# Lightning-AI/lit-llama

Hardware: NVIDIA H100
Metric: LLaMA-7B gptq.int4 decode tokens/sec (higher is better)
Workload: dtype bf16

## Files before the change

### lit-llama_b200/csrc/attention.cu

```cuda
#include <cstdlib>

#include "b2l_common.cuh"

namespace b2l {

__global__ void ring_advance_kernel(const int64_t* __restrict__ input_pos, int T, int32_t* ring_start, int S) {
  if (threadIdx.x == 0 && blockIdx.x == 0) {
    if (input_pos[T - 1] >= (int64_t)S) *ring_start = (*ring_start + 1) % S;
  }
}

__global__ void rope_append_kernel(__nv_bfloat16* __restrict__ qkv, __nv_bfloat16* __restrict__ k_cache,
                                   __nv_bfloat16* __restrict__ v_cache, const float* __restrict__ rope,
                                   const int64_t* __restrict__ input_pos, const int32_t* __restrict__ ring_start,
                                   int T, int n_head, int hs, int S, int block_size, int rope_rows) {
  const int bt = blockIdx.x, h = blockIdx.y, b = bt / T, t = bt % T;
  const int C = n_head * hs;
  long long p = input_pos ? input_pos[t] : (long long)t;
  const long long prow = rope_rows ? (long long)t : (p < block_size ? p : (long long)block_size - 1);
  __nv_bfloat16* q = qkv + (size_t)bt * 3 * C + h * hs;
  __nv_bfloat16* k = q + C;
  const __nv_bfloat16* v = q + 2 * C;
  __nv_bfloat16 *kd = k, *vd = nullptr;
  if (k_cache != nullptr) {
// ... 77 lines not shown
    } else {
#pragma unroll
      for (int e = 0; e < ATT_MAX_EPL; ++e) {
        int d = lane + 32 * e;
        kx[e] = d < hs ? bf2f(kr[d]) : 0.f;
        vx[e] = d < hs ? bf2f(vr[d]) : 0.f;
      }
    }
    float sc = 0.f;
#pragma unroll
    for (int e = 0; e < (EPL > 0 ? EPL : ATT_MAX_EPL); ++e) sc = fmaf(qv[e], kx[e], sc);
    sc = warp_sum(sc);
    const float mn = fmaxf(m, sc);
    const float corr = __expf(m - mn), pj = __expf(sc - mn);
    l = l * corr + pj;
#pragma unroll
    for (int e = 0; e < (EPL > 0 ? EPL : ATT_MAX_EPL); ++e) acc[e] = fmaf(pj, vx[e], acc[e] * corr);
    m = mn;
  }
  __shared__ float sm_m[ATT_WARPS], sm_l[ATT_WARPS];
  __shared__ float sm_acc[ATT_WARPS][32 * ATT_MAX_EPL];
  if (lane == 0) { sm_m[warp] = m; sm_l[warp] = l; }
#pragma unroll
  for (int e = 0; e < (EPL > 0 ? EPL : ATT_MAX_EPL); ++e) {
    int d = (EPL > 0) ? lane * EPL + e : lane + 32 * e;
    sm_acc[warp][d] = acc[e];
  }
  __syncthreads();
  float M = -INFINITY;
#pragma unroll
  for (int w = 0; w < ATT_WARPS; ++w) M = fmaxf(M, sm_m[w]);
  float Ls = 0.f;
  float wgt[ATT_WARPS];
#pragma unroll
  for (int w = 0; w < ATT_WARPS; ++w) {
    wgt[w] = (sm_m[w] == -INFINITY) ? 0.f : __expf(sm_m[w] - M);
    Ls += sm_l[w] * wgt[w];
  }
  if (threadIdx.x == 0) { out[0] = M; out[1] = Ls; }
  for (int d = threadIdx.x; d < hs; d += blockDim.x) {
    float a = 0.f;
#pragma unroll
    for (int w = 0; w < ATT_WARPS; ++w) a += sm_acc[w][d] * wgt[w];
    out[2 + d] = a;
  }
}

__global__ void attn_combine_kernel(const float* __restrict__ work, __nv_bfloat16* __restrict__ y, int T,
                                    int n_head, int hs, int n_split) {
  pdl_launch_dependents();
  const int bh = blockIdx.x, b = bh / n_head, h = bh % n_head, t = blockIdx.y;
  const float* base = work + ((size_t)bh * T + t) * n_split * (hs + 2);
  float M = -INFINITY;
  for (int s = 0; s < n_split; ++s) M = fmaxf(M, base[(size_t)s * (hs + 2)]);
  float Ls = 0.f;
  for (int s = 0; s < n_split; ++s) {
    float ms = base[(size_t)s * (hs + 2)];
    if (ms != -INFINITY) Ls += base[(size_t)s * (hs + 2) + 1] * __expf(ms - M);
  }
  const float inv = 1.0f / Ls;
  __nv_bfloat16* yr = y + ((size_t)b * T + t) * (n_head * hs) + h * hs;
  for (int d = threadIdx.x; d < hs; d += blockDim.x) {
    float a = 0.f;
    for (int s = 0; s < n_split; ++s) {
      float ms = base[(size_t)s * (hs + 2)];
      if (ms != -INFINITY) a += base[(size_t)s * (hs + 2) + 2 + d] * __expf(ms - M);
    }
    yr[d] = f2bf(a * inv);
  }
}

__global__ void kv_unroll_kernel(const __nv_bfloat16* __restrict__ cache, const int32_t* __restrict__ ring_start,
                                 __nv_bfloat16* __restrict__ out, int S, int hs) {
  const int ring = *ring_start;
  const int phys = (blockIdx.y + ring) % S;
  const __nv_bfloat16* src = cache + ((size_t)blockIdx.x * S + phys) * hs;
  __nv_bfloat16* dst = out + ((size_t)blockIdx.x * S + blockIdx.y) * hs;
  for (int d = threadIdx.x; d < hs; d += blockDim.x) dst[d] = src[d];
}

constexpr int FD_CHUNK = 256;
constexpr int FD_SUB = 64;
constexpr int FD_WARPS = 8;
constexpr int FD_CTAS_PER_SM = 3;
constexpr int WS_CHUNK = FD_SUB;

__device__ __forceinline__ void bf16x8_to_f32(const uint4& u, float* f) {
  const uint32_t w[4] = {u.x, u.y, u.z, u.w};
#pragma unroll
  for (int i = 0; i < 4; ++i) {
    f[2 * i] = __uint_as_float(w[i] << 16);
    f[2 * i + 1] = __uint_as_float(w[i] & 0xffff0000u);
  }
}

__device__ __forceinline__ uint32_t fd_smem_u32(const void* p) { return (uint32_t)__cvta_generic_to_shared(p); }
__device__ __forceinline__ void fd_bulk(uint32_t dst, const void* src, uint32_t bytes, uint32_t bar) {
  asm volatile("cp.async.bulk.shared::cluster.global.mbarrier::complete_tx::bytes [%0], [%1], %2, [%3];" ::"r"(dst), "l"(src), "r"(bytes), "r"(bar) : "memory");
}

constexpr int FD_SUB_BYTES = FD_SUB * 128 * 2;
constexpr int FD_SMEM_BYTES = 4 * FD_SUB_BYTES + FD_WARPS * 128 * 4 + 2 * FD_WARPS * 4 + 16;

__global__ void __launch_bounds__(FD_WARPS * 32)
    attn_decode_fused_kernel(const __nv_bfloat16* qkv, __nv_bfloat16* __restrict__ k_cache,
                             __nv_bfloat16* __restrict__ v_cache, const float* __restrict__ rope,
                             const int64_t* __restrict__ input_pos, const int32_t* __restrict__ ring_start,
                             __nv_bfloat16* __restrict__ y, float* __restrict__ work, int* __restrict__ tickets,
                             int n_head, int S, int block_size, int n_split, unsigned long long* tl, int pre_tiles,
                             int smem_merge, int target_ctas) {
  constexpr int HS = 128;
  extern __shared__ __align__(128) uint8_t fsm[];
  float* sm_acc = reinterpret_cast<float*>(fsm + 4 * FD_SUB_BYTES);
  float* sm_m = sm_acc + FD_WARPS * HS;
  float* sm_l = sm_m + FD_WARPS;
  unsigned long long* bars = reinterpret_cast<unsigned long long*>(sm_l + FD_WARPS);
  __shared__ int sm_last;

  if (threadIdx.x == 0) tl_min(tl, 0);
  const int bh = blockIdx.x, b = bh / n_head, h = bh % n_head, sp = blockIdx.y;
  unsigned long long* tl0 = (tl != nullptr && blockIdx.x == 0 && blockIdx.y == 0 && threadIdx.x == 0) ? tl + 8 : nullptr;
  int tli = 0;
  auto stamp = [&]() { if (tl0 != nullptr && tli < 24) tl0[tli++] = globaltimer_ns(); };
  stamp();
  const int lane = threadIdx.x & 31, warp = threadIdx.x >> 5;
  const int C = n_head * HS;
  const size_t head_base = ((size_t)b * n_head + h) * S * HS;

  const long long p = input_pos[0];
  const int w_slot = (int)(p < S ? p : (long long)S - 1);
  const int L = w_slot + 1;
  const int want_splits = max(1, target_ctas / (int)gridDim.x);
  const int chunk = L <= FD_CHUNK ? FD_CHUNK
                                  : min(FD_CHUNK, max(FD_SUB, FD_SUB * ((L + FD_SUB * want_splits - 1) / (FD_SUB * want_splits))));
  const int n_active = (L + chunk - 1) / chunk;
  if (sp >= n_active) return;
  const int ring = *ring_start;
  const int j0 = sp * chunk, j1 = min(L, j0 + chunk);
  const int n_old = min(j1, L - 1) - j0;
  const int n_sub = (n_old + FD_SUB - 1) / FD_SUB;
  const bool has_new = (w_slot >= j0 && w_slot < j1);

  const uint32_t bar0 = fd_smem_u32(bars);
  auto request = [&](int i) {
    const int buf = i & 1;
    const int cnt = min(FD_SUB, n_old - i * FD_SUB);
    int phys0 = j0 + i * FD_SUB + ring; if (phys0 >= S) phys0 -= S;
    const int first = min(cnt, S - phys0);
    const uint32_t bar = bar0 + buf * 8;
    const uint32_t kd = fd_smem_u32(fsm) + buf * 2 * FD_SUB_BYTES, vd = kd + FD_SUB_BYTES;
    asm volatile("mbarrier.arrive.expect_tx.shared::cta.b64 _, [%0], %1;" ::"r"(bar), "r"((uint32_t)cnt * HS * 2 * 2) : "memory");
    fd_bulk(kd, k_cache + head_base + (size_t)phys0 * HS, (uint32_t)first * HS * 2, bar);
    fd_bulk(vd, v_cache + head_base + (size_t)phys0 * HS, (uint32_t)first * HS * 2, bar);
    if (first < cnt) {
      fd_bulk(kd + first * HS * 2, k_cache + head_base, (uint32_t)(cnt - first) * HS * 2, bar);
      fd_bulk(vd + first * HS * 2, v_cache + head_base, (uint32_t)(cnt - first) * HS * 2, bar);
    }
  };
  const int pre = (n_active == 1) ? 2 : pre_tiles;
  if (threadIdx.x == 0) {
    asm volatile("mbarrier.init.shared::cta.b64 [%0], 1;" ::"r"(bar0) : "memory");
    asm volatile("mbarrier.init.shared::cta.b64 [%0], 1;" ::"r"(bar0 + 8) : "memory");
    asm volatile("fence.mbarrier_init.release.cluster;" ::: "memory");
    if (n_sub > 0) request(0);
    if (pre > 1 && n_sub > 1) request(1);
  }
  const long long prow = p < block_size ? p : (long long)block_size - 1;
  const int grp = lane >> 3, sub = lane & 7, d0 = sub * 16;
  float cs[16];
  {
    const float4* rp = reinterpret_cast<const float4*>(rope + ((size_t)prow * (HS / 2) + d0 / 2) * 2);
#pragma unroll
    for (int i = 0; i < 4; ++i) {
      float4 t = rp[i];
      cs[4 * i] = t.x; cs[4 * i + 1] = t.y; cs[4 * i + 2] = t.z; cs[4 * i + 3] = t.w;
    }
  }
  __syncthreads();
  pdl_wait();
  if (threadIdx.x == 0) tl_max(tl, 1);
  stamp();
  pdl_launch_dependents();

  const __nv_bfloat16* qrow = qkv + (size_t)b * 3 * C + h * HS + d0;
  float q[16];
  {
    float raw[16];
    const uint4 qa = ld_coherent_u4(qrow), qb = ld_coherent_u4(qrow + 8);
    if (threadIdx.x == 0 && pre <= 1 && n_sub > 1) request(1);
    bf16x8_to_f32(qa, raw);
    bf16x8_to_f32(qb, raw + 8);
    const float scale = rsqrtf((float)HS);
#pragma unroll
    for (int i = 0; i < 8; ++i) {
      const float c = cs[2 * i], s_ = cs[2 * i + 1];
      const float e = rbf(__fsub_rn(__fmul_rn(raw[2 * i], c), __fmul_rn(raw[2 * i + 1], s_)));
      const float o = rbf(__fadd_rn(__fmul_rn(raw[2 * i + 1], c), __fmul_rn(raw[2 * i], s_)));
      q[2 * i] = e * scale;
      q[2 * i + 1] = o * scale;
    }
  }

  float m = -INFINITY, l = 0.f, acc[16];
#pragma unroll
  for (int i = 0; i < 16; ++i) acc[i] = 0.f;
  if (tl0 != nullptr && q[0] != 12345.678f) stamp();
  if (has_new && warp == 0 && grp == 0) {
    int phys = w_slot + ring; if (phys >= S) phys -= S;
    float raw[16], kf[16], vf[16];
    bf16x8_to_f32(ld_coherent_u4(qrow + C), raw);
    bf16x8_to_f32(ld_coherent_u4(qrow + C + 8), raw + 8);
    uint32_t out[8];
#pragma unroll
    for (int i = 0; i < 8; ++i) {
      const float c = cs[2 * i], s_ = cs[2 * i + 1];
      kf[2 * i] = rbf(__fsub_rn(__fmul_rn(raw[2 * i], c), __fmul_rn(raw[2 * i + 1], s_)));
      kf[2 * i + 1] = rbf(__fadd_rn(__fmul_rn(raw[2 * i + 1], c), __fmul_rn(raw[2 * i], s_)));
      out[i] = (__float_as_uint(kf[2 * i]) >> 16) | (__float_as_uint(kf[2 * i + 1]) & 0xffff0000u);
    }
    const uint4 va = ld_coherent_u4(qrow + 2 * C), vb = ld_coherent_u4(qrow + 2 * C + 8);
    uint4* kd = reinterpret_cast<uint4*>(k_cache + head_base + (size_t)phys * HS + d0);
    uint4* vd = reinterpret_cast<uint4*>(v_cache + head_base + (size_t)phys * HS + d0);
    kd[0] = make_uint4(out[0], out[1], out[2], out[3]); kd[1] = make_uint4(out[4], out[5], out[6], out[7]);
    vd[0] = va; vd[1] = vb;
    bf16x8_to_f32(va, vf); bf16x8_to_f32(vb, vf + 8);
    float sc = 0.f;
#pragma unroll
    for (int e = 0; e < 16; ++e) sc = fmaf(q[e], kf[e], sc);
    sc += __shfl_xor_sync(0x000000ffu, sc, 1);
    sc += __shfl_xor_sync(0x000000ffu, sc, 2);
    sc += __shfl_xor_sync(0x000000ffu, sc, 4);
    const float mn = fmaxf(m, sc);
    const float corr = __expf(m - mn), pj = __expf(sc - mn);
    l = l * corr + pj;
#pragma unroll
    for (int e = 0; e < 16; ++e) acc[e] = fmaf(pj, vf[e], acc[e] * corr);
    m = mn;
  }
  for (int i = 0; i < n_sub; ++i) {
    const int buf = i & 1;
    const int cnt = min(FD_SUB, n_old - i * FD_SUB);
    {
      uint32_t ok;
      const uint32_t par = (uint32_t)(i >> 1) & 1u;
      do {
        asm volatile("{\n\t.reg .pred p;\n\tmbarrier.try_wait.parity.shared::cta.b64 p, [%1], %2;\n\tselp.u32 %0, 1, 0, p;\n\t}" : "=r"(ok) : "r"(bar0 + buf * 8), "r"(par) : "memory");
      } while (!ok);
    }
    const __nv_bfloat16* kt = reinterpret_cast<const __nv_bfloat16*>(fsm + buf * 2 * FD_SUB_BYTES);
    const __nv_bfloat16* vt = kt + FD_SUB * HS;
    stamp();
    float sc[2];
    bool valid[2];
    const uint4* vr[2];
#pragma unroll
    for (int it = 0; it < 2; ++it) {
      const int r = warp * 8 + it * 4 + grp;
      valid[it] = r < cnt;
      const int rc = valid[it] ? r : 0;
      const uint4* kr = reinterpret_cast<const uint4*>(kt + (size_t)rc * HS + d0);
      vr[it] = reinterpret_cast<const uint4*>(vt + (size_t)rc * HS + d0);
      float kf[16];
      bf16x8_to_f32(kr[0], kf); bf16x8_to_f32(kr[1], kf + 8);
      float a0 = 0.f, a1 = 0.f;
#pragma unroll
      for (int e = 0; e < 8; ++e) { a0 = fmaf(q[e], kf[e], a0); a1 = fmaf(q[8 + e], kf[8 + e], a1); }
      sc[it] = a0 + a1;
    }
#pragma unroll
    for (int o = 1; o <= 4; o <<= 1) {
      sc[0] += __shfl_xor_sync(0xffffffffu, sc[0], o);
      sc[1] += __shfl_xor_sync(0xffffffffu, sc[1], o);
    }
    {
      const float s0 = valid[0] ? sc[0] : -INFINITY, s1 = valid[1] ? sc[1] : -INFINITY;
      const float mn = fmaxf(m, fmaxf(s0, s1));
      if (mn != -INFINITY) {
        const float corr = __expf(m - mn), p0 = __expf(s0 - mn), p1 = __expf(s1 - mn);
        float v0[16], v1[16];
        bf16x8_to_f32(vr[0][0], v0); bf16x8_to_f32(vr[0][1], v0 + 8);
        bf16x8_to_f32(vr[1][0], v1); bf16x8_to_f32(vr[1][1], v1 + 8);
        l = l * corr + p0 + p1;
#pragma unroll
        for (int e = 0; e < 16; ++e) acc[e] = fmaf(p1, v1[e], fmaf(p0, v0[e], acc[e] * corr));
        m = mn;
      }
    }
    __syncthreads();
    stamp();
    if (threadIdx.x == 0 && i + 2 < n_sub) request(i + 2);
  }
  if (threadIdx.x == 0) tl_max(tl, 2);
  __syncwarp();
  if (threadIdx.x == 0) tl_max(tl, 3);
  float* part = reinterpret_cast<float*>(fsm);
  float* pm = part + 32 * HS;
  float* pl = pm + 32, *pw = pl + 32;
  const int n_part = smem_merge ? 32 : FD_WARPS;
  if (smem_merge) {
    const int g = warp * 4 + grp;
    float4* dst = reinterpret_cast<float4*>(part + g * HS + d0);
#pragma unroll
    for (int i = 0; i < 4; ++i) dst[i] = make_float4(acc[4 * i], acc[4 * i + 1], acc[4 * i + 2], acc[4 * i + 3]);
    if (sub == 0) { pm[g] = m; pl[g] = l; }
  } else {
#pragma unroll
    for (int off = 8; off <= 16; off <<= 1) {
      const float mo = __shfl_xor_sync(0xffffffffu, m, off);
      const float lo = __shfl_xor_sync(0xffffffffu, l, off);
      const float mn = fmaxf(m, mo);
      const float ca = (m == -INFINITY) ? 0.f : __expf(m - mn);
      const float cb = (mo == -INFINITY) ? 0.f : __expf(mo - mn);
      l = l * ca + lo * cb;
#pragma unroll
      for (int i = 0; i < 16; ++i) {
        const float ao = __shfl_xor_sync(0xffffffffu, acc[i], off);
        acc[i] = acc[i] * ca + ao * cb;
      }
      m = mn;
    }
    if (lane == 0) { pm[warp] = m; pl[warp] = l; }
    if (grp == 0) {
      float4* dst = reinterpret_cast<float4*>(part + warp * HS + d0);
#pragma unroll
      for (int i = 0; i < 4; ++i) dst[i] = make_float4(acc[4 * i], acc[4 * i + 1], acc[4 * i + 2], acc[4 * i + 3]);
    }
  }
  __syncthreads();
  if (warp == 0) {
    const float mi = lane < n_part ? pm[lane] : -INFINITY;
    const float Mx = warp_max(mi);
    const float wi = (mi == -INFINITY) ? 0.f : __expf(mi - Mx);
    const float Lx = warp_sum(lane < n_part ? pl[lane] * wi : 0.f);
    pw[lane] = wi;
    if (lane == 0) { pw[32] = Mx; pw[33] = Lx; }
  }
  __syncthreads();
  const float M = pw[32], Ls = pw[33];
  const int d = threadIdx.x & (HS - 1);
  const bool writer = threadIdx.x < HS;
  float a = 0.f;
  if (writer) {
#pragma unroll 8
    for (int g = 0; g < n_part; ++g) a = fmaf(part[g * HS + d], pw[g], a);
  }
  stamp();
  if (n_active == 1) {
    if (writer) y[(size_t)b * C + h * HS + d] = f2bf(a / Ls);
    if (threadIdx.x == 0) tl_max(tl, 4);
    stamp();
    return;
  }
  float* out = work + ((size_t)bh * n_split + sp) * (HS + 2);
  if (threadIdx.x == 0) { out[0] = M; out[1] = Ls; }
  if (writer) out[2 + d] = a;
  __syncthreads();
  if (threadIdx.x == 0) {
    int t;
    asm volatile("atom.add.acq_rel.gpu.global.s32 %0, [%1], 1;" : "=r"(t) : "l"(tickets + bh) : "memory");
    sm_last = (t == n_active - 1);
    if (sm_last) tickets[bh] = 0;
  }
  __syncthreads();
  stamp();
  if (!sm_last) return;
  const float* base = work + (size_t)bh * n_split * (HS + 2);
  float MM = -INFINITY, LL = 0.f, aa = 0.f;
  for (int s0 = 0; s0 < n_active; s0 += 8) {
    float ms[8], ls[8], as[8];
#pragma unroll
    for (int i = 0; i < 8; ++i) {
      const int s2 = s0 + i;
      const bool ok = s2 < n_active;
// ... 185 lines not shown
  }
#pragma unroll
  for (int r = 0; r < 2; ++r) {
    lrow[r] += __shfl_xor_sync(0xffffffffu, lrow[r], 1);
    lrow[r] += __shfl_xor_sync(0xffffffffu, lrow[r], 2);
  }
#pragma unroll
  for (int r = 0; r < 2; ++r) {
    const int t = t0 + warp * 16 + g + 8 * r;
    if (t < T) {
      const float inv = 1.0f / lrow[r];
      __nv_bfloat16* dst = y + ((size_t)b * T + t) * C + h * HS + 2 * t4;
#pragma unroll
      for (int n = 0; n < 16; ++n)
        *reinterpret_cast<__nv_bfloat162*>(dst + n * 8) = __floats2bfloat162_rn(o[n][2 * r] * inv, o[n][2 * r + 1] * inv);
    }
  }
}

void* g_attn_timeline = nullptr;

static inline void split_plan(int T, int S, int* n_split, int* chunk) {
  if (T > 1) { *n_split = 1; *chunk = S; return; }
  *chunk = 64;
  *n_split = (S + 63) / 64;
}

static int launch_attn(const __nv_bfloat16* qkv, KvView kv, const int64_t* input_pos, const int32_t* ring_start,
                       float* work, __nv_bfloat16* y, int B, int T, int n_head, int hs, int cap, cudaStream_t st) {
  static const int env_pf = [] { const char* e = getenv("B2L_ATTN_PREFILL"); return e ? atoi(e) : 1; }();
  if (hs == 128 && T > 1 && env_pf) {
    static DynSmemCache smem_cache;
    if (int rc = ensure_dyn_smem(attn_prefill_kernel, PF_SMEM_BYTES, smem_cache)) return rc;
    attn_prefill_kernel<<<dim3(B * n_head, (T + PF_Q - 1) / PF_Q), 128, PF_SMEM_BYTES, st>>>(qkv, kv, input_pos, ring_start, y, T, n_head);
    B2L_LAUNCH_CHECK("attn_prefill_kernel");
    return 0;
  }
  int n_split, chunk;
  split_plan(T, cap, &n_split, &chunk);
  dim3 grid(B * n_head, T, n_split), block(ATT_WARPS * 32);
  if (hs == 128)
    attn_partial_kernel<4><<<grid, block, 0, st>>>(qkv, kv, input_pos, ring_start, work, T, n_head, hs, n_split, chunk);
  else
    attn_partial_kernel<0><<<grid, block, 0, st>>>(qkv, kv, input_pos, ring_start, work, T, n_head, hs, n_split, chunk);
  B2L_LAUNCH_CHECK("attn_partial_kernel");
  attn_combine_kernel<<<dim3(B * n_head, T), 128, 0, st>>>(work, y, T, n_head, hs, n_split);
  B2L_LAUNCH_CHECK("attn_combine_kernel");
  return 0;
}

}

using namespace b2l;

static inline size_t ws_partials_bytes(int B, int n_head, int head_size, int T, int S) {
  int n_split, chunk;
  split_plan(T, S, &n_split, &chunk);
  size_t a = (size_t)B * n_head * T * n_split * (head_size + 2) * sizeof(float);
  size_t f = (size_t)B * n_head * ((S + WS_CHUNK - 1) / WS_CHUNK) * (head_size + 2) * sizeof(float);
  return ((a > f ? a : f) + 15) & ~(size_t)15;
}

extern "C" size_t b2l_attn_workspace_bytes(int B, int n_head, int head_size, int T, int S) {
  return ws_partials_bytes(B, n_head, head_size, T, S) + (size_t)B * n_head * sizeof(int);
}

extern "C" int b2l_ring_advance(const int64_t* input_pos, int T, int32_t* ring_start, int S, b2l_stream_t stream) {
  B2L_CHECK_ARG(input_pos && ring_start && T > 0 && S > 0, "b2l_ring_advance: bad argument");
  ring_advance_kernel<<<1, 32, 0, (cudaStream_t)stream>>>(input_pos, T, ring_start, S);
  B2L_LAUNCH_CHECK("ring_advance_kernel");
  return 0;
}

extern "C" int b2l_attention(void* qkv, void* k_cache, void* v_cache, const void* rope, const int64_t* input_pos,
                             const int32_t* ring_start, void* y, void* work, int B, int T, int n_head,
                             int head_size, int S, int block_size, int flags, b2l_stream_t stream) {
  B2L_CHECK_ARG(qkv && k_cache && v_cache && rope && input_pos && ring_start && y && work,
                "b2l_attention: null pointer");
  B2L_CHECK_ARG(B > 0 && T > 0 && n_head > 0 && S > 0 && T <= S && block_size > 0, "b2l_attention: bad shape");
  B2L_CHECK_SUPPORTED(head_size % 2 == 0 && head_size >= 2 && head_size <= 32 * ATT_MAX_EPL,
                      "b2l_attention: head_size %d unsupported (even, <= %d)", head_size, 32 * ATT_MAX_EPL);
  cudaStream_t st = (cudaStream_t)stream;
  if (T == 1 && head_size == 128 && !(flags & B2L_F_ROPE_ROWS) && !(flags & B2L_F_ATTN_UNFUSED)) {
    const int n_split = (S + FD_SUB - 1) / FD_SUB;
    int* tickets = reinterpret_cast<int*>(reinterpret_cast<char*>(work) + ws_partials_bytes(B, n_head, head_size, T, S));
    static DynSmemCache smem_cache;
    static const int env_pre = [] { const char* e = getenv("B2L_ATTN_PRE"); return e ? atoi(e) : 1; }();
    static const int env_smem_merge = [] { const char* e = getenv("B2L_ATTN_SMEM_MERGE"); return e ? atoi(e) : 0; }();
    if (int rc = ensure_dyn_smem(attn_decode_fused_kernel, FD_SMEM_BYTES, smem_cache)) return rc;
    LaunchCfg lc(dim3(B * n_head, n_split), dim3(FD_WARPS * 32), FD_SMEM_BYTES, st, (flags & B2L_F_PDL) != 0);
    B2L_CUDA(cudaLaunchKernelEx(&lc.cfg, attn_decode_fused_kernel, (const __nv_bfloat16*)qkv, (__nv_bfloat16*)k_cache,
                                (__nv_bfloat16*)v_cache, (const float*)rope, input_pos, ring_start, (__nv_bfloat16*)y,
                                (float*)work, tickets, n_head, S, block_size, n_split, (unsigned long long*)g_attn_timeline, env_pre, env_smem_merge,
                                FD_CTAS_PER_SM * sm_count()));
    return 0;
  }
  int rt = head_size / 2 < 32 ? 32 : head_size / 2;
  rope_append_kernel<<<dim3(B * T, n_head), rt, 0, st>>>((__nv_bfloat16*)qkv, (__nv_bfloat16*)k_cache,
                                                        (__nv_bfloat16*)v_cache, (const float*)rope, input_pos,
                                                        ring_start, T, n_head, head_size, S, block_size, (flags & B2L_F_ROPE_ROWS) ? 1 : 0);
  B2L_LAUNCH_CHECK("rope_append_kernel");
  KvView kv{(const __nv_bfloat16*)k_cache, (const __nv_bfloat16*)v_cache, (size_t)n_head * S * head_size,
            (size_t)S * head_size, (size_t)head_size, S};
  return launch_attn((const __nv_bfloat16*)qkv, kv, input_pos, ring_start, (float*)work, (__nv_bfloat16*)y, B, T,
                     n_head, head_size, S, st);
}

extern "C" int b2l_attention_nocache(void* qkv, const void* rope, void* y, void* work, int B, int T, int n_head,
                                     int head_size, int block_size, b2l_stream_t stream) {
  B2L_CHECK_ARG(qkv && rope && y && work && B > 0 && T > 0 && n_head > 0 && T <= block_size,
                "b2l_attention_nocache: bad argument");
  B2L_CHECK_SUPPORTED(head_size % 2 == 0 && head_size >= 2 && head_size <= 32 * ATT_MAX_EPL,
                      "b2l_attention_nocache: head_size %d unsupported", head_size);
  cudaStream_t st = (cudaStream_t)stream;
  int rt = head_size / 2 < 32 ? 32 : head_size / 2;
  rope_append_kernel<<<dim3(B * T, n_head), rt, 0, st>>>((__nv_bfloat16*)qkv, nullptr, nullptr, (const float*)rope,
                                                        nullptr, nullptr, T, n_head, head_size, 0, block_size, 0);
  B2L_LAUNCH_CHECK("rope_append_kernel");
  const int C = n_head * head_size;
  const __nv_bfloat16* base = (const __nv_bfloat16*)qkv;
  KvView kv{base + C, base + 2 * C, (size_t)T * 3 * C, (size_t)head_size, (size_t)3 * C, 0};
  return launch_attn(base, kv, nullptr, nullptr, (float*)work, (__nv_bfloat16*)y, B, T, n_head, head_size, T, st);
}

extern "C" int b2l_kv_unroll(const void* cache, const int32_t* ring_start, void* out, int B, int n_head, int S,
                             int head_size, b2l_stream_t stream) {
  B2L_CHECK_ARG(cache && ring_start && out && B > 0 && n_head > 0 && S > 0 && head_size > 0,
                "b2l_kv_unroll: bad argument");
  kv_unroll_kernel<<<dim3(B * n_head, S), 64, 0, (cudaStream_t)stream>>>((const __nv_bfloat16*)cache, ring_start,
                                                                         (__nv_bfloat16*)out, S, head_size);
  B2L_LAUNCH_CHECK("kv_unroll_kernel");
  return 0;
}
```

### lit-llama_b200/csrc/b2l_common.cuh

```cuda
#pragma once
#include <cuda_bf16.h>
#include <cuda_runtime.h>
#include <stdint.h>

#include <cstdarg>
#include <cstdio>

#include "../../include/b2l.h"

#if defined(__CUDA_ARCH__) && (__CUDA_ARCH__ != 900)
#error "libb200llama is written for sm_90a (H100) only"
#endif

namespace b2l {

void set_error(const char* fmt, ...);
int cuda_fail(cudaError_t e, const char* what);

#define B2L_CHECK_ARG(cond, ...)                  \
  do {                                            \
    if (!(cond)) {                                \
      b2l::set_error(__VA_ARGS__);                \
      return B2L_E_ARG;                           \
    }                                             \
  } while (0)
#define B2L_CHECK_SUPPORTED(cond, ...)            \
  do {                                            \
    if (!(cond)) {                                \
      b2l::set_error(__VA_ARGS__);                \
      return B2L_E_UNSUPPORTED;                   \
    }                                             \
  } while (0)
#define B2L_CUDA(call)                                          \
  do {                                                          \
    cudaError_t e_ = (call);                                    \
    if (e_ != cudaSuccess) return b2l::cuda_fail(e_, #call);    \
  } while (0)
#define B2L_LAUNCH_CHECK(name)                                       \
  do {                                                               \
    cudaError_t e_ = cudaGetLastError();                             \
    if (e_ != cudaSuccess) return b2l::cuda_fail(e_, "launch " name); \
  } while (0)

int sm_count();

constexpr int B2L_MAX_DEVICES = 64;
struct DynSmemCache {
  size_t bytes[B2L_MAX_DEVICES] = {};
};
template <typename Kernel>
inline int ensure_dyn_smem(Kernel kernel, size_t bytes, DynSmemCache& cache) {
  int dev = 0;
  B2L_CUDA(cudaGetDevice(&dev));
  if (dev < 0 || dev >= B2L_MAX_DEVICES) {
    B2L_CUDA(cudaFuncSetAttribute(kernel, cudaFuncAttributeMaxDynamicSharedMemorySize, (int)bytes));
    return 0;
  }
  if (bytes > cache.bytes[dev]) {
    B2L_CUDA(cudaFuncSetAttribute(kernel, cudaFuncAttributeMaxDynamicSharedMemorySize, (int)bytes));
    cache.bytes[dev] = bytes;
  }
  return 0;
}

__device__ __forceinline__ float bf2f(__nv_bfloat16 v) { return __bfloat162float(v); }
__device__ __forceinline__ __nv_bfloat16 f2bf(float v) { return __float2bfloat16_rn(v); }
__device__ __forceinline__ float rbf(float v) { return __bfloat162float(__float2bfloat16_rn(v)); }

__device__ __forceinline__ float load_sz(const void* p, int dtype, size_t i) {
  return dtype == B2L_BF16 ? bf2f(reinterpret_cast<const __nv_bfloat16*>(p)[i])
                           : reinterpret_cast<const float*>(p)[i];
}

__device__ __forceinline__ float warp_sum(float v) {
#pragma unroll
  for (int o = 16; o > 0; o >>= 1) v += __shfl_xor_sync(0xffffffffu, v, o);
  return v;
}
__device__ __forceinline__ float warp_max(float v) {
#pragma unroll
  for (int o = 16; o > 0; o >>= 1) v = fmaxf(v, __shfl_xor_sync(0xffffffffu, v, o));
  return v;
}

__device__ __forceinline__ float block_sum(float v, float* red) {
  const int lane = threadIdx.x & 31, warp = threadIdx.x >> 5, nw = (blockDim.x + 31) >> 5;
  v = warp_sum(v);
  __syncthreads();
  if (lane == 0) red[warp] = v;
  __syncthreads();
  float t = (lane < nw) ? red[lane] : 0.f;
  return warp_sum(t);
}

__device__ __forceinline__ unsigned long long globaltimer_ns() {
  unsigned long long t;
  asm volatile("mov.u64 %0, %%globaltimer;" : "=l"(t));
  return t;
}
__device__ __forceinline__ void tl_min(unsigned long long* tr, int slot) {
  if (tr != nullptr) atomicMin(tr + slot, globaltimer_ns());
}
__device__ __forceinline__ void tl_max(unsigned long long* tr, int slot) {
  if (tr != nullptr) atomicMax(tr + slot, globaltimer_ns());
}

__device__ __forceinline__ void pdl_wait() { asm volatile("griddepcontrol.wait;" ::: "memory"); }
__device__ __forceinline__ void pdl_launch_dependents() {
  asm volatile("griddepcontrol.launch_dependents;" ::: "memory");
}

__device__ __forceinline__ uint4 ld_coherent_u4(const void* p) {
  uint4 v;
  asm volatile("ld.global.v4.u32 {%0, %1, %2, %3}, [%4];" : "=r"(v.x), "=r"(v.y), "=r"(v.z), "=r"(v.w) : "l"(p) : "memory");
  return v;
}

__device__ __forceinline__ float rms_rinv(float sumsq, int C, float eps) {
  float ms = rbf(sumsq / (float)C);
  float t = rbf(ms + eps);
  return rbf(1.0f / sqrtf(t));
}
__device__ __forceinline__ float rms_apply(float x, float rinv, float scale) {
  return rbf(scale * rbf(x * rinv));
}

struct LaunchCfg {
  cudaLaunchConfig_t cfg;
  cudaLaunchAttribute attrs[2];
  LaunchCfg(dim3 grid, dim3 block, size_t smem, cudaStream_t stream, bool pdl, int cluster_x = 1) {
    cfg = cudaLaunchConfig_t{};
    cfg.gridDim = grid;
    cfg.blockDim = block;
    cfg.dynamicSmemBytes = smem;
    cfg.stream = stream;
    int n = 0;
    if (pdl) {
      attrs[n].id = cudaLaunchAttributeProgrammaticStreamSerialization;
      attrs[n].val.programmaticStreamSerializationAllowed = 1;
// ... 16 lines not shown
```

### lit-llama_b200/csrc/q4_gemv.cu

```cuda
#include <cstdlib>

#include "q4_mma_common.cuh"

namespace b2l {
namespace q4mv {

struct Params {
  const __nv_bfloat16* x;
  const uint8_t* qwt;
  const void* scales; const void* zeros; int szdt;
  __nv_bfloat16* y;
  int N, K;
  int n_rb;
  int prologue; const __nv_bfloat16* norm_scale; float eps;
  int epilogue; const __nv_bfloat16* res;
  int nst;
  unsigned long long* tl;
  int nocompute;
  const uint8_t* pf_ptr[B2L_PF_SEGMENTS];
  uint32_t pf_bytes[B2L_PF_SEGMENTS];
  int pf_mode;
  const uint8_t* pf_kv[2]; const long long* pf_rows; int pf_rows_max, pf_nseg, pf_row_bytes; unsigned long long pf_seg_stride;
  int evict_first;
};

constexpr uint32_t PF_CHUNK = 16384;

__host__ __device__ inline uint32_t plane_stride(int K) { return (uint32_t)K + ((K % 128 == 0) ? 64u : 0u); }

struct SmemLayout {
  uint32_t ring, xf, zero, scratch, red, sxp, bars, total;
};
__host__ __device__ inline SmemLayout smem_layout(int nst, int K, int ndig) {
  SmemLayout L;
  uint32_t o = 0;
  L.ring = o;    o += (uint32_t)nst * STAGE_BYTES;
  L.xf = o;      o += (uint32_t)ndig * plane_stride(K);
  L.zero = o;    o += 16;
  L.scratch = o; o += 2 * NCW * MAX_HALVES * RB * 16;
  L.red = o;     o += 192;
  L.sxp = o;     o += NCW * 32 * 4;
  L.bars = o;    o += 2 * MAX_STAGES * 8;
  L.total = (o + 127u) & ~127u;
  return L;
}

__device__ __forceinline__ void l2_prefetch_bulk(const void* src, uint32_t bytes) {
  asm volatile("cp.async.bulk.prefetch.L2.global [%0], %1;" ::"l"(src), "r"(bytes) : "memory");
}
__device__ __forceinline__ void l2_prefetch_line(const void* src) {
  asm volatile("prefetch.global.L2 [%0];" ::"l"(src));
}
__device__ __forceinline__ void pf_slice(uint32_t bytes, uint32_t& lo, uint32_t& hi) {
  const uint32_t lines = (bytes + 127u) >> 7;
  lo = (uint32_t)(((unsigned long long)blockIdx.x * lines) / gridDim.x) << 7;
  hi = min((uint32_t)(((unsigned long long)(blockIdx.x + 1) * lines) / gridDim.x) << 7, bytes);
}
__device__ __forceinline__ void tma_bulk_g2s_hint(uint32_t dst, const void* src, uint32_t bytes, uint32_t mbar, uint64_t policy) {
  asm volatile(
      "cp.async.bulk.shared::cluster.global.mbarrier::complete_tx::bytes.L2::cache_hint [%0], [%1], %2, [%3], %4;" ::"r"(dst),
      "l"(src), "r"(bytes), "r"(mbar), "l"(policy)
      : "memory");
}

__device__ __forceinline__ uint32_t balanced_digits(int X) { return ((uint32_t)X + 0x00808080u) ^ 0x00808080u; }

template <int NH>
__device__ __forceinline__ void kblock_imma(int (&acc)[MAX_HALVES][2][4], const uint8_t* wbase, const uint4& xb) {
#pragma unroll
  for (int h = 0; h < NH; ++h) {
    const uint4 wv = *reinterpret_cast<const uint4*>(wbase + h * HALF_STAGE_BYTES);
    mma_u8s8_16832(acc[h][0], wv.x, wv.x & 0xf0f0f0f0u, wv.y, wv.y & 0xf0f0f0f0u, xb.x, xb.y);
    mma_u8s8_16832(acc[h][1], wv.z, wv.z & 0xf0f0f0f0u, wv.w, wv.w & 0xf0f0f0f0u, xb.z, xb.w);
  }
}

__device__ __forceinline__ void single_imma(int (&a)[2][4], const uint8_t* tile, const uint4& xb) {
  const uint4 wv = *reinterpret_cast<const uint4*>(tile);
  mma_u8s8_16832(a[0], wv.x, wv.x & 0xf0f0f0f0u, wv.y, wv.y & 0xf0f0f0f0u, xb.x, xb.y);
  mma_u8s8_16832(a[1], wv.z, wv.z & 0xf0f0f0f0u, wv.w, wv.w & 0xf0f0f0f0u, xb.z, xb.w);
}

template <int MAXC, int NDIG>
__global__ void __launch_bounds__(NTHREADS, 2) q4_gemv_kernel(const Params p) {
  extern __shared__ __align__(128) uint8_t smem[];
  const SmemLayout L = smem_layout(p.nst, p.K, NDIG);
  const uint32_t sbase = smem_u32(smem);
  const int tid = threadIdx.x, warp = tid >> 5, lane = tid & 31;
  const int n_kb = p.K / KB;
  const int spu2 = (n_kb + KBP_PER_STAGE - 1) / KBP_PER_STAGE, spu1 = (n_kb + 2 * KBP_PER_STAGE - 1) / (2 * KBP_PER_STAGE);
  const int rb_lo = (int)(((long long)blockIdx.x * p.n_rb) / gridDim.x);
  const int rb_hi = (int)(((long long)(blockIdx.x + 1) * p.n_rb) / gridDim.x);
  const int n_units = (rb_hi - rb_lo + 1) / 2;
  const int total_stages = ((rb_hi - rb_lo) / 2) * spu2 + ((rb_hi - rb_lo) & 1) * spu1;
  const uint32_t bar_full = sbase + L.bars, bar_empty = bar_full + MAX_STAGES * 8;
  const uint32_t PS = plane_stride(p.K);

  if (tid == 0) tl_min(p.tl, 0);
  if (tid == 0) {
    for (int i = 0; i < p.nst; ++i) {
      mbar_init(bar_full + i * 8, 1);
      mbar_init(bar_empty + i * 8, NCW);
    }
    asm volatile("fence.mbarrier_init.release.cluster;" ::: "memory");
  }
  if (tid < 4) reinterpret_cast<uint32_t*>(smem + L.zero)[tid] = 0u;
  __syncthreads();

  if (warp == PRODUCER_WARP) {
    if (lane == 0) {
      int slot = 0;
      uint32_t phase = 1;
      int it = 0;
      uint64_t policy = 0;
      if (p.evict_first) asm volatile("createpolicy.fractional.L2::evict_first.b64 %0, 1.0;" : "=l"(policy));
      for (int u = 0; u < n_units; ++u) {
        const int rb = rb_lo + 2 * u;
        const int halves = min(2, rb_hi - rb);
        const uint8_t* src = p.qwt + (size_t)rb * n_kb * KB_BYTES;
        const int per_stage = halves == 2 ? KBP_PER_STAGE : 2 * KBP_PER_STAGE;
        for (int kb0 = 0; kb0 < n_kb; kb0 += per_stage, ++it) {
          const int nkb = min(per_stage, n_kb - kb0);
          const uint32_t bytes = (uint32_t)nkb * KB_BYTES;
          mbar_wait(bar_empty + slot * 8, phase);
          mbar_expect_tx(bar_full + slot * 8, bytes * halves);
          for (int h = 0; h < halves; ++h) {
            const uint32_t dst = sbase + L.ring + slot * STAGE_BYTES + h * HALF_STAGE_BYTES;
            const uint8_t* from = src + ((size_t)h * n_kb + kb0) * KB_BYTES;
            if (p.evict_first) tma_bulk_g2s_hint(dst, from, bytes, bar_full + slot * 8, policy);
            else tma_bulk_g2s(dst, from, bytes, bar_full + slot * 8);
          }
          if (++slot == p.nst) { slot = 0; phase ^= 1; }
          if (it + 1 == min(total_stages, p.nst)) {
            pdl_launch_dependents();
            if (p.pf_mode == 1) {
#pragma unroll
              for (int sgi = 0; sgi < B2L_PF_SEGMENTS; ++sgi) {
                if (p.pf_bytes[sgi] == 0) continue;
                uint32_t lo, hi;
                pf_slice(p.pf_bytes[sgi], lo, hi);
#pragma unroll 1
                for (uint32_t o = lo; o < hi; o += PF_CHUNK) l2_prefetch_bulk(p.pf_ptr[sgi] + o, min(PF_CHUNK, hi - o));
              }
            }
          }
        }
      }
      if (total_stages == 0) pdl_launch_dependents();
      if (p.pf_kv[0] != nullptr) {
        long long rows = *p.pf_rows;
        rows = rows < 0 ? 0 : (rows > p.pf_rows_max ? p.pf_rows_max : rows);
        const uint32_t seg_bytes = (uint32_t)rows * (uint32_t)p.pf_row_bytes;
        const uint32_t cps = (seg_bytes + PF_CHUNK - 1) / PF_CHUNK;
        const uint32_t total = 2u * (uint32_t)p.pf_nseg * cps;
#pragma unroll 1
        for (uint32_t id = blockIdx.x; id < total; id += gridDim.x) {
          const uint32_t sg = id / cps, o = (id - sg * cps) * PF_CHUNK;
          const uint32_t which = sg >= (uint32_t)p.pf_nseg ? 1u : 0u;
          const uint8_t* base = p.pf_kv[which] + (size_t)(sg - which * p.pf_nseg) * p.pf_seg_stride;
          l2_prefetch_bulk(base + o, min(PF_CHUNK, seg_bytes - o));
        }
      }
    }
  } else if (warp < NCW) {
    float* red = reinterpret_cast<float*>(smem + L.red);
    int* red_sh = reinterpret_cast<int*>(smem + L.red + 128);
    {
      const bool norm = (p.prologue == B2L_PRO_RMSNORM);
      constexpr int NT = NCW * 32;
      constexpr uint32_t MAGIC_BITS = 0x4B400000u;
      uint4 xv[MAXC], gv[MAXC];
      __nv_bfloat162 gmax2 = __float2bfloat162_rn(0.f);
#pragma unroll
      for (int c = 0; c < MAXC; ++c) {
        const int k = (c * NT + tid) * 8;
        gv[c] = make_uint4(0, 0, 0, 0);
        if (norm && k < p.K) gv[c] = *reinterpret_cast<const uint4*>(p.norm_scale + k);
      }
      if (norm) {
#pragma unroll
        for (int c = 0; c < MAXC; ++c) {
// ... 293 lines not shown
using namespace b2l::q4mv;

extern "C" size_t b2l_q4_tiled_i8_bytes(int N, int K) {
  if (N <= 0 || K <= 0 || K % KB != 0) return 0;
  return (size_t)((N + RB - 1) / RB) * (K / KB) * KB_BYTES;
}

extern "C" int b2l_q4_tile_i8(const void* qw, void* qw_tiled, int N, int K, b2l_stream_t stream) {
  B2L_CHECK_ARG(qw && qw_tiled && N > 0 && K > 0, "b2l_q4_tile_i8: bad argument");
  B2L_CHECK_SUPPORTED(K % KB == 0, "b2l_q4_tile_i8: in_features %d must be a multiple of %d", K, KB);
  const size_t total = b2l_q4_tiled_i8_bytes(N, K) / 4;
  q4_tile_i8_kernel<<<(unsigned)((total + 255) / 256), 256, 0, (cudaStream_t)stream>>>((const uint8_t*)qw, (uint32_t*)qw_tiled, N, K);
  B2L_LAUNCH_CHECK("q4_tile_i8_kernel");
  return 0;
}

extern "C" int b2l_q4_untile_i8(const void* qw_tiled, void* qw, int N, int K, b2l_stream_t stream) {
  B2L_CHECK_ARG(qw && qw_tiled && N > 0 && K > 0, "b2l_q4_untile_i8: bad argument");
  B2L_CHECK_SUPPORTED(K % KB == 0, "b2l_q4_untile_i8: in_features %d must be a multiple of %d", K, KB);
  const size_t total = (size_t)(K / 2) * N;
  q4_untile_i8_kernel<<<(unsigned)((total + 255) / 256), 256, 0, (cudaStream_t)stream>>>((const uint32_t*)qw_tiled, (uint8_t*)qw, N, K);
  B2L_LAUNCH_CHECK("q4_untile_i8_kernel");
  return 0;
}

namespace {
constexpr int MAX_K = 12 * NCW * 32 * 8;

template <int MAXC, int NDIG>
int launch_gemv(const Params& p0, int ctas_per_sm, int grid_override, bool pdl, cudaStream_t stream) {
  Params p = p0;
  static const int env_kb = [] { const char* e = getenv("B2L_GEMV_SMEM_KB"); return e ? atoi(e) : 0; }();
  const uint32_t budget = (env_kb > 0 ? (uint32_t)env_kb : (ctas_per_sm >= 2 ? 110u : 224u)) * 1024u;
  const uint32_t fixed = smem_layout(0, p.K, NDIG).total;
  int nst = fixed + 2 * STAGE_BYTES <= budget ? (int)((budget - fixed) / STAGE_BYTES) : 0;
  if (nst > MAX_STAGES) nst = MAX_STAGES;
  static const int env_nst = [] { const char* e = getenv("B2L_GEMV_STAGES"); return e ? atoi(e) : 0; }();
  if (env_nst > 0 && nst > env_nst) nst = env_nst;
  if (nst < 2) {
    set_error("b2l_q4_gemv: K=%d does not leave room for the weight ring", p.K);
    return B2L_E_UNSUPPORTED;
  }
  p.nst = nst;
  const SmemLayout L = smem_layout(nst, p.K, NDIG);
  static DynSmemCache smem_cache;
  if (int rc = ensure_dyn_smem(q4_gemv_kernel<MAXC, NDIG>, L.total, smem_cache)) return rc;
  int grid = grid_override > 0 ? grid_override : ctas_per_sm * sm_count();
  if (grid > p.n_rb) grid = p.n_rb;
  LaunchCfg lc(dim3(grid), dim3(NTHREADS), L.total, stream, pdl, 1);
  B2L_CUDA(cudaLaunchKernelEx(&lc.cfg, q4_gemv_kernel<MAXC, NDIG>, p));
  return 0;
}
}

extern "C" int b2l_q4_gemv(const b2l_q4_linear_args* a, b2l_stream_t stream) {
  B2L_CHECK_ARG(a != nullptr, "b2l_q4_gemv: null args");
  B2L_CHECK_ARG(a->x && a->qw_tiled && a->scales && a->zeros && a->y, "b2l_q4_gemv: null pointer");
  B2L_CHECK_SUPPORTED(a->M == 1, "b2l_q4_gemv: M=%d (this kernel is the batch-1 path; use b2l_q4_gemv_batch / b2l_q4_linear_tc)", a->M);
  B2L_CHECK_SUPPORTED(a->K > 0 && a->K % KB == 0 && a->K <= MAX_K, "b2l_q4_gemv: K=%d must be a multiple of %d and <= %d", a->K, KB, MAX_K);
  B2L_CHECK_ARG(a->N > 0, "b2l_q4_gemv: bad N");
  B2L_CHECK_ARG(((uintptr_t)a->x % 16 == 0) && ((uintptr_t)a->qw_tiled % 16 == 0), "b2l_q4_gemv: x / qw_tiled must be 16-byte aligned");
  B2L_CHECK_ARG(a->sz_dtype == B2L_BF16 || a->sz_dtype == B2L_F32, "b2l_q4_gemv: bad sz_dtype");
  if (a->prologue == B2L_PRO_RMSNORM)
    B2L_CHECK_ARG(a->norm_scale && ((uintptr_t)a->norm_scale % 16 == 0), "b2l_q4_gemv: RMSNorm prologue needs a 16-byte aligned scale");
  else
    B2L_CHECK_ARG(a->prologue == B2L_PRO_NONE, "b2l_q4_gemv: bad prologue %d", a->prologue);
  if (a->epilogue == B2L_EPI_RESIDUAL) B2L_CHECK_ARG(a->res != nullptr, "b2l_q4_gemv: RESIDUAL epilogue needs res");
  else if (a->epilogue == B2L_EPI_SWIGLU) B2L_CHECK_SUPPORTED(a->N % RB == 0, "b2l_q4_gemv: SWIGLU needs N %% 16 == 0");
  else B2L_CHECK_ARG(a->epilogue == B2L_EPI_STORE, "b2l_q4_gemv: bad epilogue %d", a->epilogue);

  Params p;
  p.x = (const __nv_bfloat16*)a->x;
  p.qwt = (const uint8_t*)a->qw_tiled;
  p.scales = a->scales; p.zeros = a->zeros; p.szdt = a->sz_dtype;
  p.y = (__nv_bfloat16*)a->y;
  p.N = a->N; p.K = a->K;
  p.n_rb = (a->N + RB - 1) / RB;
  p.prologue = a->prologue; p.norm_scale = (const __nv_bfloat16*)a->norm_scale; p.eps = a->eps;
  p.epilogue = a->epilogue; p.res = (const __nv_bfloat16*)a->res;
  p.nst = 0;
  p.tl = (unsigned long long*)a->trace;
  p.nocompute = (a->flags & B2L_F_DEBUG_NOCOMPUTE) ? 1 : 0;
  static const int env_pf_mode = [] { const char* e = getenv("B2L_PF_MODE"); return e ? atoi(e) : 1; }();
  static const int env_evict = [] { const char* e = getenv("B2L_PF_EVICT"); return e ? atoi(e) : 0; }();
  p.pf_mode = 0;
  p.evict_first = env_evict;
  p.pf_kv[0] = p.pf_kv[1] = nullptr; p.pf_rows = nullptr; p.pf_rows_max = p.pf_nseg = p.pf_row_bytes = 0; p.pf_seg_stride = 0;
  if (a->pf_kv[0] != nullptr) {
    B2L_CHECK_ARG(a->pf_kv[1] != nullptr && a->pf_rows != nullptr && a->pf_rows_max > 0 && a->pf_nseg > 0 && a->pf_row_bytes > 0 &&
                      a->pf_row_bytes % 16 == 0 && a->pf_seg_stride % 16 == 0 && ((uintptr_t)a->pf_kv[0] % 16 == 0) &&
                      ((uintptr_t)a->pf_kv[1] % 16 == 0) && (unsigned long long)a->pf_rows_max * a->pf_row_bytes < (1ull << 31),
                  "b2l_q4_gemv: bad strided prefetch hint");
    p.pf_kv[0] = (const uint8_t*)a->pf_kv[0]; p.pf_kv[1] = (const uint8_t*)a->pf_kv[1];
    p.pf_rows = a->pf_rows; p.pf_rows_max = a->pf_rows_max; p.pf_nseg = a->pf_nseg; p.pf_row_bytes = a->pf_row_bytes;
    p.pf_seg_stride = a->pf_seg_stride;
  }
  for (int i = 0; i < B2L_PF_SEGMENTS; ++i) {
    p.pf_ptr[i] = (const uint8_t*)a->pf_ptr[i];
    p.pf_bytes[i] = 0;
    if (a->pf_ptr[i] != nullptr && a->pf_bytes[i] != 0) {
      B2L_CHECK_ARG(((uintptr_t)a->pf_ptr[i] % 16 == 0) && (a->pf_bytes[i] % 16 == 0) && a->pf_bytes[i] < (1ull << 31),
                    "b2l_q4_gemv: prefetch segment %d must be 16-byte aligned, a multiple of 16 and < 2 GiB", i);
      p.pf_bytes[i] = (uint32_t)a->pf_bytes[i];
      p.pf_mode = env_pf_mode;
    }
  }
  static const int env_cps = [] { const char* e = getenv("B2L_GEMV_CTAS_PER_SM"); return e ? atoi(e) : 0; }();
  const bool pdl = (a->flags & B2L_F_PDL) != 0;
  cudaStream_t st = (cudaStream_t)stream;
  const int grid = a->split_k;
  if (a->K <= 12288) return launch_gemv<6, 3>(p, env_cps > 0 ? env_cps : 2, grid, pdl, st);
  if (a->K <= 16384) return launch_gemv<12, 3>(p, env_cps > 0 ? env_cps : 2, grid, pdl, st);
  return launch_gemv<12, 3>(p, 1, grid, pdl, st);
}
```

Baseline: 581.9.

## Use fewer, larger attention splits with triple-buffered KV loads and evict-first weights

The default decode-attention launch now sizes the split count so there is about one CTA per SM (chunks up to 512 positions) and uses three bulk-copy buffers instead of two, giving deeper prefetch of K/V tiles. The shared-memory carveout is set to max-shared so the larger buffers fit, and launch bounds allow two CTAs per SM. The GEMV weight stream now uses an L2 evict_first policy by default, aiming to keep KV and activations resident in L2. Fewer splits mean less merge work but also less parallelism for short contexts.

```diff
diff --git a/lit-llama_b200/csrc/attention.cu b/lit-llama_b200/csrc/attention.cu
--- a/lit-llama_b200/csrc/attention.cu
+++ b/lit-llama_b200/csrc/attention.cu
@@ -183,7 +183,8 @@
 constexpr int FD_CHUNK = 256;
 constexpr int FD_SUB = 64;
 constexpr int FD_WARPS = 8;
-constexpr int FD_CTAS_PER_SM = 3;
+constexpr int FD_MAX_CHUNK = 512;
+constexpr int FD_MAX_BUF = 3;
 constexpr int WS_CHUNK = FD_SUB;
 
 __device__ __forceinline__ void bf16x8_to_f32(const uint4& u, float* f) {
@@ -201,24 +202,24 @@
 }
 
 constexpr int FD_SUB_BYTES = FD_SUB * 128 * 2;
-constexpr int FD_SMEM_BYTES = 4 * FD_SUB_BYTES + FD_WARPS * 128 * 4 + 2 * FD_WARPS * 4 + 16;
-
-__global__ void __launch_bounds__(FD_WARPS * 32)
+constexpr int fd_smem_bytes(int nbuf) { return nbuf * 2 * FD_SUB_BYTES + FD_WARPS * 128 * 4 + 2 * FD_WARPS * 4 + nbuf * 8; }
+
+__global__ void __launch_bounds__(FD_WARPS * 32, 2)
     attn_decode_fused_kernel(const __nv_bfloat16* qkv, __nv_bfloat16* __restrict__ k_cache,
                              __nv_bfloat16* __restrict__ v_cache, const float* __restrict__ rope,
                              const int64_t* __restrict__ input_pos, const int32_t* __restrict__ ring_start,
                              __nv_bfloat16* __restrict__ y, float* __restrict__ work, int* __restrict__ tickets,
                              int n_head, int S, int block_size, int n_split, unsigned long long* tl, int pre_tiles,
-                             int smem_merge, int target_ctas) {
+                             int smem_merge, int want_splits, int max_chunk, int nbuf) {
   constexpr int HS = 128;
   extern __shared__ __align__(128) uint8_t fsm[];
-  float* sm_acc = reinterpret_cast<float*>(fsm + 4 * FD_SUB_BYTES);
+  float* sm_acc = reinterpret_cast<float*>(fsm + nbuf * 2 * FD_SUB_BYTES);
   float* sm_m = sm_acc + FD_WARPS * HS;
   float* sm_l = sm_m + FD_WARPS;
   unsigned long long* bars = reinterpret_cast<unsigned long long*>(sm_l + FD_WARPS);
   __shared__ int sm_last;
 
-  if (threadIdx.x == 0) tl_min(tl, 0);
+  if (threadIdx.x == 0) { tl_min(tl, 0); tl_max(tl, 5); }
   const int bh = blockIdx.x, b = bh / n_head, h = bh % n_head, sp = blockIdx.y;
   unsigned long long* tl0 = (tl != nullptr && blockIdx.x == 0 && blockIdx.y == 0 && threadIdx.x == 0) ? tl + 8 : nullptr;
   int tli = 0;
@@ -231,9 +232,8 @@
   const long long p = input_pos[0];
   const int w_slot = (int)(p < S ? p : (long long)S - 1);
   const int L = w_slot + 1;
-  const int want_splits = max(1, target_ctas / (int)gridDim.x);
   const int chunk = L <= FD_CHUNK ? FD_CHUNK
-                                  : min(FD_CHUNK, max(FD_SUB, FD_SUB * ((L + FD_SUB * want_splits - 1) / (FD_SUB * want_splits))));
+                                  : min(max_chunk, max(FD_SUB, FD_SUB * ((L + FD_SUB * want_splits - 1) / (FD_SUB * want_splits))));
   const int n_active = (L + chunk - 1) / chunk;
   if (sp >= n_active) return;
   const int ring = *ring_start;
@@ -244,7 +244,7 @@
 
   const uint32_t bar0 = fd_smem_u32(bars);
   auto request = [&](int i) {
-    const int buf = i & 1;
+    const int buf = i % nbuf;
     const int cnt = min(FD_SUB, n_old - i * FD_SUB);
     int phys0 = j0 + i * FD_SUB + ring; if (phys0 >= S) phys0 -= S;
     const int first = min(cnt, S - phys0);
@@ -258,13 +258,11 @@
       fd_bulk(vd + first * HS * 2, v_cache + head_base, (uint32_t)(cnt - first) * HS * 2, bar);
     }
   };
-  const int pre = (n_active == 1) ? 2 : pre_tiles;
+  const int pre = min(nbuf, (n_active == 1) ? 2 : pre_tiles);
   if (threadIdx.x == 0) {
-    asm volatile("mbarrier.init.shared::cta.b64 [%0], 1;" ::"r"(bar0) : "memory");
-    asm volatile("mbarrier.init.shared::cta.b64 [%0], 1;" ::"r"(bar0 + 8) : "memory");
+    for (int i = 0; i < nbuf; ++i) asm volatile("mbarrier.init.shared::cta.b64 [%0], 1;" ::"r"(bar0 + i * 8) : "memory");
     asm volatile("fence.mbarrier_init.release.cluster;" ::: "memory");
-    if (n_sub > 0) request(0);
-    if (pre > 1 && n_sub > 1) request(1);
+    for (int i = 0; i < min(pre, n_sub); ++i) request(i);
   }
   const long long prow = p < block_size ? p : (long long)block_size - 1;
   const int grp = lane >> 3, sub = lane & 7, d0 = sub * 16;
@@ -288,7 +286,8 @@
   {
     float raw[16];
     const uint4 qa = ld_coherent_u4(qrow), qb = ld_coherent_u4(qrow + 8);
-    if (threadIdx.x == 0 && pre <= 1 && n_sub > 1) request(1);
+    if (threadIdx.x == 0)
+      for (int i = pre; i < min(nbuf, n_sub); ++i) request(i);
     bf16x8_to_f32(qa, raw);
     bf16x8_to_f32(qb, raw + 8);
     const float scale = rsqrtf((float)HS);
@@ -339,11 +338,11 @@
     m = mn;
   }
   for (int i = 0; i < n_sub; ++i) {
-    const int buf = i & 1;
+    const int buf = i % nbuf;
     const int cnt = min(FD_SUB, n_old - i * FD_SUB);
     {
       uint32_t ok;
-      const uint32_t par = (uint32_t)(i >> 1) & 1u;
+      const uint32_t par = (uint32_t)(i / nbuf) & 1u;
       do {
         asm volatile("{\n\t.reg .pred p;\n\tmbarrier.try_wait.parity.shared::cta.b64 p, [%1], %2;\n\tselp.u32 %0, 1, 0, p;\n\t}" : "=r"(ok) : "r"(bar0 + buf * 8), "r"(par) : "memory");
       } while (!ok);
@@ -389,7 +388,7 @@
     }
     __syncthreads();
     stamp();
-    if (threadIdx.x == 0 && i + 2 < n_sub) request(i + 2);
+    if (threadIdx.x == 0 && i + nbuf < n_sub) request(i + nbuf);
   }
   if (threadIdx.x == 0) tl_max(tl, 2);
   __syncwarp();
@@ -741,17 +740,31 @@
                       "b2l_attention: head_size %d unsupported (even, <= %d)", head_size, 32 * ATT_MAX_EPL);
   cudaStream_t st = (cudaStream_t)stream;
   if (T == 1 && head_size == 128 && !(flags & B2L_F_ROPE_ROWS) && !(flags & B2L_F_ATTN_UNFUSED)) {
-    const int n_split = (S + FD_SUB - 1) / FD_SUB;
+    static const int env_cps = [] { const char* e = getenv("B2L_ATTN_CTAS_PER_SM"); return e ? atoi(e) : 1; }();
+    const int max_split = (S + FD_SUB - 1) / FD_SUB;
+    int n_split, want_splits, max_chunk, nbuf;
+    if (env_cps >= 3) {
+      n_split = max_split;
+      want_splits = max(1, 3 * sm_count() / (B * n_head));
+      max_chunk = FD_CHUNK;
+      nbuf = 2;
+    } else {
+      n_split = min(max_split, max(sm_count() / (B * n_head), (S + FD_MAX_CHUNK - 1) / FD_MAX_CHUNK));
+      want_splits = n_split;
+      max_chunk = FD_MAX_CHUNK;
+      nbuf = FD_MAX_BUF;
+    }
+    const int smem = fd_smem_bytes(nbuf);
     int* tickets = reinterpret_cast<int*>(reinterpret_cast<char*>(work) + ws_partials_bytes(B, n_head, head_size, T, S));
     static DynSmemCache smem_cache;
     static const int env_pre = [] { const char* e = getenv("B2L_ATTN_PRE"); return e ? atoi(e) : 1; }();
     static const int env_smem_merge = [] { const char* e = getenv("B2L_ATTN_SMEM_MERGE"); return e ? atoi(e) : 0; }();
-    if (int rc = ensure_dyn_smem(attn_decode_fused_kernel, FD_SMEM_BYTES, smem_cache)) return rc;
-    LaunchCfg lc(dim3(B * n_head, n_split), dim3(FD_WARPS * 32), FD_SMEM_BYTES, st, (flags & B2L_F_PDL) != 0);
+    if (int rc = ensure_dyn_smem(attn_decode_fused_kernel, smem, smem_cache)) return rc;
+    LaunchCfg lc(dim3(B * n_head, n_split), dim3(FD_WARPS * 32), smem, st, (flags & B2L_F_PDL) != 0);
     B2L_CUDA(cudaLaunchKernelEx(&lc.cfg, attn_decode_fused_kernel, (const __nv_bfloat16*)qkv, (__nv_bfloat16*)k_cache,
                                 (__nv_bfloat16*)v_cache, (const float*)rope, input_pos, ring_start, (__nv_bfloat16*)y,
                                 (float*)work, tickets, n_head, S, block_size, n_split, (unsigned long long*)g_attn_timeline, env_pre, env_smem_merge,
-                                FD_CTAS_PER_SM * sm_count()));
+                                want_splits, max_chunk, nbuf));
     return 0;
   }
   int rt = head_size / 2 < 32 ? 32 : head_size / 2;
diff --git a/lit-llama_b200/csrc/b2l_common.cuh b/lit-llama_b200/csrc/b2l_common.cuh
--- a/lit-llama_b200/csrc/b2l_common.cuh
+++ b/lit-llama_b200/csrc/b2l_common.cuh
@@ -47,14 +47,20 @@
 constexpr int B2L_MAX_DEVICES = 64;
 struct DynSmemCache {
   size_t bytes[B2L_MAX_DEVICES] = {};
+  bool carveout[B2L_MAX_DEVICES] = {};
 };
 template <typename Kernel>
 inline int ensure_dyn_smem(Kernel kernel, size_t bytes, DynSmemCache& cache) {
   int dev = 0;
   B2L_CUDA(cudaGetDevice(&dev));
   if (dev < 0 || dev >= B2L_MAX_DEVICES) {
+    B2L_CUDA(cudaFuncSetAttribute(kernel, cudaFuncAttributePreferredSharedMemoryCarveout, (int)cudaSharedmemCarveoutMaxShared));
     B2L_CUDA(cudaFuncSetAttribute(kernel, cudaFuncAttributeMaxDynamicSharedMemorySize, (int)bytes));
     return 0;
+  }
+  if (!cache.carveout[dev]) {
+    B2L_CUDA(cudaFuncSetAttribute(kernel, cudaFuncAttributePreferredSharedMemoryCarveout, (int)cudaSharedmemCarveoutMaxShared));
+    cache.carveout[dev] = true;
   }
   if (bytes > cache.bytes[dev]) {
     B2L_CUDA(cudaFuncSetAttribute(kernel, cudaFuncAttributeMaxDynamicSharedMemorySize, (int)bytes));
diff --git a/lit-llama_b200/csrc/q4_gemv.cu b/lit-llama_b200/csrc/q4_gemv.cu
--- a/lit-llama_b200/csrc/q4_gemv.cu
+++ b/lit-llama_b200/csrc/q4_gemv.cu
@@ -96,7 +96,7 @@
   const uint32_t bar_full = sbase + L.bars, bar_empty = bar_full + MAX_STAGES * 8;
   const uint32_t PS = plane_stride(p.K);
 
-  if (tid == 0) tl_min(p.tl, 0);
+  if (tid == 0) { tl_min(p.tl, 0); tl_max(p.tl, 5); }
   if (tid == 0) {
     for (int i = 0; i < p.nst; ++i) {
       mbar_init(bar_full + i * 8, 1);
@@ -556,7 +556,7 @@
   p.tl = (unsigned long long*)a->trace;
   p.nocompute = (a->flags & B2L_F_DEBUG_NOCOMPUTE) ? 1 : 0;
   static const int env_pf_mode = [] { const char* e = getenv("B2L_PF_MODE"); return e ? atoi(e) : 1; }();
-  static const int env_evict = [] { const char* e = getenv("B2L_PF_EVICT"); return e ? atoi(e) : 0; }();
+  static const int env_evict = [] { const char* e = getenv("B2L_PF_EVICT"); return e ? atoi(e) : 1; }();
   p.pf_mode = 0;
   p.evict_first = env_evict;
   p.pf_kv[0] = p.pf_kv[1] = nullptr; p.pf_rows = nullptr; p.pf_rows_max = p.pf_nseg = p.pf_row_bytes = 0; p.pf_seg_stride = 0;
```

After: 581.9, median of 6. No clear change (+0.0%).
